# zyang1580/PDA

Hardware: AMD Instinct MI355X
Metric: users/sec full-catalogue top-K@50 (eval) (higher is better)
Workload: dtype f32; 1 GPU; C3: synthetic 1000000 users x 200000 items, d=128, PDA condition ((elu+1)*pop^0.22) head, masked top-K@50; ranks_seen=1

## Files before the change

pda_amd/csrc/pda_score_topk_v4.hip:

```cpp
#include "pda_v4_shared.h"
#include <cstdlib>
#include <type_traits>

using namespace pda_topk;

namespace {

constexpr int kCap4 = 57;
constexpr int kRing4 = 128;
constexpr int kWarmTiles = 4;
constexpr int kMainWaves = 8;
#ifndef PDA_W4_ABL
#define PDA_W4_ABL 0
#endif
#ifdef PDA_V4_PROF
__device__ unsigned long long pda_prof4[24];
#define PROF_T0(v) const long long v = __builtin_readcyclecounter()
#define PROF_T1(v, slot) prof[slot] += (unsigned long long)(__builtin_readcyclecounter() - v)
#define PROF_INC(slot, x) prof[slot] += (unsigned long long)(x)
#define PROF_FLUSH(first, last) do { if (lane == 0) for (int pq = (first); pq <= (last); ++pq) atomicAdd(&pda_prof4[pq], prof[pq]); } while (0)
#else
#define PROF_T0(v) do {} while (0)
#define PROF_T1(v, slot) do {} while (0)
#define PROF_INC(slot, x) do {} while (0)
// ... 634 lines not shown
            if (needa) ta = mna;
            if (needb) tb = mnb;
            for (int it = 0; it < 40; ++it) {
                const bool opena = needa && ca_t > cap_t && hia - ta > 1u;
                const bool openb = needb && cb_t > cap_t && hib - tb > 1u;
                if (!__any(opena || openb)) break;
                const uint32_t mida = opena ? ta + ((hia - ta) >> 1) : ta;
                const uint32_t midb = openb ? tb + ((hib - tb) >> 1) : tb;
                int cnta, cntb;
                count_ge2(mida, midb, cnta, cntb);
                if (opena) {
                    if (cnta >= K) {
                        ta = mida;
                        ca_t = cnta;
                    } else {
                        hia = mida;
                    }
                }
                if (openb) {
                    if (cntb >= K) {
                        tb = midb;
                        cb_t = cntb;
                    } else {
                        hib = midb;
                    }
                }
            }
        }
        emit_row(r, ta, ca_t);
        emit_row(r + 1, tb, cb_t);
    }
    pda_wave_sync();
    if (tid == 0) atomicAdd(reinterpret_cast<unsigned long long*>(g.stats + 2), (unsigned long long)(2 * nwarm));
    for (int rr = 0; rr < 32; ++rr) {
        uint64_t* buf = my_lists + rr * CAP;
        if (((PDA_W4_ABL & 4) == 0) && (g.warm_sorted || g.warm_final || (g.handover == nullptr && __builtin_amdgcn_readfirstlane(cntl[wave * 32 + rr]) > K)))
            compact_list<CAP>(buf, &cntl[wave * 32 + rr], &taul[wave * 32 + rr], K, lane);
        const int c = cntl[wave * 32 + rr];
        const int rb = utile * kUserTile + wave * 32 + rr;
        if (g.seed_out != nullptr) {
            uint32_t mn = lane < c ? (uint32_t)(buf[lane] >> 32) : 0xFFFFFFFFu;
#pragma unroll
            for (int o = 32; o >= 1; o >>= 1) mn = min(mn, (uint32_t)__shfl_xor((int)mn, o, 64));
            if (lane == 0 && rb < g.n_users_blk) g.seed_out[rb] = c >= K ? pda_unordf(mn) : -INFINITY;
        }
        if (g.kth_ws != nullptr) continue;
        if (g.handover != nullptr) {
            if (rb < g.n_users_blk && lane < CAP) g.handover[((size_t)split * g.n_users_blk + rb) * CAP + lane] = lane < c ? buf[lane] : 0ull;
            if (g.warm_final && rb < g.n_users_blk && lane < K) g.out_keys[((size_t)split * g.n_users_blk + rb) * K + lane] = lane < c ? buf[lane] : 0ull;
        } else if (rb < g.n_users_blk && lane < K) {
            const uint64_t k = lane < c ? buf[lane] : 0ull;
            g.out_keys[((size_t)split * g.n_users_blk + rb) * K + lane] = k;
        }
    }
    if (g.kth_ws != nullptr) {
        pda_wave_sync();
        const int rb0 = utile * kUserTile + wave * 32, nv = max(0, min(32, g.n_users_blk - rb0));
        if (lane < nv) {
            const uint64_t kl = my_lists[(size_t)lane * CAP + (K - 1)];
            g.kth_ws[(size_t)split * g.n_users_blk + rb0 + lane] = cntl[wave * 32 + lane] >= K ? pda_unordf((uint32_t)(kl >> 32)) : -INFINITY;
        }
        uint64_t* ob = g.out_keys + ((size_t)split * g.n_users_blk + rb0) * K;
        const int q64 = 64 / K, r64 = 64 % K;
        int rr = lane / K, p = lane % K;
        for (int i = lane; i < nv * K; i += 64) {
            ob[i] = p < cntl[wave * 32 + rr] ? my_lists[(size_t)rr * CAP + p] : 0ull;
            rr += q64;
            p += r64;
            if (p >= K) { p -= K; ++rr; }
        }
    }
    if (g.pred_ws != nullptr && lane < 32) {
        const int rb = utile * kUserTile + wave * 32 + lane;
        if (rb < g.n_users_blk) {
            g.pred_ws[2 * (size_t)rb] = predt[wave * 32 + lane];
            g.pred_ws[2 * (size_t)rb + 1] = nul[wave * 32 + lane];
        }
    }
}

constexpr int kWS5Waves = 8, kWS5Threads = 64 * kWS5Waves;
constexpr int kWarmPos = 64 * kWarmTiles;
constexpr size_t warm_score5_lds(int d) { return (size_t)kWarmPos * d * 4 + kWarmPos * 8 + (size_t)kWS5Waves * 32 * 2 * kWarmTiles * 4; }

template <int D, bool BF>
__global__ void __launch_bounds__(kWS5Threads) warm_score5_kernel(Args4 g) {
    extern __shared__ __attribute__((aligned(16))) unsigned char smem[];
    constexpr int RB = row_bytes(D);
    constexpr int NC = D / 8;
    constexpr int CPR4 = D / 4;
    float* Bt = reinterpret_cast<float*>(smem);
    float* popw = Bt + kWarmPos * D;
    int* idw = reinterpret_cast<int*>(popw + kWarmPos);
    unsigned* hmask = reinterpret_cast<unsigned*>(idw + kWarmPos);

    const int tid = threadIdx.x, lane = tid & 63, wave = tid >> 6;
    const int j = lane & 31, h = lane >> 5;
    const int nwarm = g.warm_tiles;
    const int npos = 64 * nwarm;
    for (int p = tid; p < npos; p += kWS5Threads) {
        const float* tl = reinterpret_cast<const float*>(g.rows + (size_t)p * RB + 2 * D + 32);
        popw[p] = tl[0];
        idw[p] = reinterpret_cast<const int*>(tl)[1];
    }
    __syncthreads();
    for (int id = tid; id < npos * CPR4; id += kWS5Threads) {
        const int jj = id / CPR4, ch = id % CPR4;
        *reinterpret_cast<f32x4*>(Bt + jj * D + 4 * (ch ^ swz<D>(jj & 31))) = pda_load4<BF>(g.I, (size_t)idw[jj] * D + 4 * ch);
    }
    if (blockIdx.x == 0) {
        for (int p = tid; p < kWarmPos; p += kWS5Threads) g.wscore[p] = p < npos ? (uint32_t)idw[p] : 0u;
        if (tid == 0) g.stats[8] = 5u;
    }
    __syncthreads();

    uint32_t* scores = g.wscore + kWarmPos;
    const int utiles_w = (g.n_users_blk + kUserTile - 1) / kUserTile;
    const int nunits = utiles_w * (kUserTile / 32);
    const int G = (int)gridDim.x, stride = G * kWS5Waves;
    unsigned* hm_l = hmask + wave * 32 * 2 * kWarmTiles;
    static_assert(2 * kWarmTiles == 8, "two 16-byte loads per row");

    auto row_uid = [&](int unit) -> int {
        const int rb = unit * 32 + j;
        return (unit < nunits && rb < g.n_users_blk) ? g.users[rb] : 0;
    };
    auto load_rows = [&](int unit_x, int uid, f32x4 (&a)[NC], u32x4& hm, bool& hm_on) __attribute__((always_inline)) {
        if (unit_x >= nunits) return;
        const int rb = unit_x * 32 + j;
#pragma unroll
        for (int c = 0; c < NC; ++c) a[c] = pda_load4<BF>(g.U, (size_t)uid * D + 4 * h + 8 * c);
        hm_on = false;
        if (g.hmask_tab != nullptr) {
            hm_on = rb < g.n_users_blk && (unsigned)uid < (unsigned)g.hmask_tab_rows;
            hm = *reinterpret_cast<const u32x4*>(g.hmask_tab + (size_t)(hm_on ? uid : 0) * (2 * kWarmTiles) + 4 * h);
        } else if (g.hmask_ws != nullptr) {
            hm_on = true;
            hm = *reinterpret_cast<const u32x4*>(g.hmask_ws + (size_t)rb * (2 * kWarmTiles) + 4 * h);
        }
    };
    unsigned long long n_tiles_done = 0ull;
    auto run_unit = [&](const int unit_in, f32x4 (&areg)[NC], const u32x4& hm_in, const bool hm_on) __attribute__((always_inline)) {
        const int unit = __builtin_amdgcn_readfirstlane(unit_in);
        const int row_blk = unit * 32 + j;
        if (unit * 32 + 32 > g.n_users_blk) {
            const f32x4 z = {0.f, 0.f, 0.f, 0.f};
#pragma unroll
            for (int c = 0; c < NC; ++c) areg[c] = row_blk < g.n_users_blk ? areg[c] : z;
        }
        const u32x4 hz = {0u, 0u, 0u, 0u};
        const u32x4 hmv = hm_on ? hm_in : hz;
        *reinterpret_cast<u32x4*>(hm_l + j * (2 * kWarmTiles) + 4 * h) = hmv;
        {
            constexpr int NK5 = D / 32;
            unsigned char* fb = g.ufrag_out + ((size_t)(row_blk >> 4) * (NK5 * 64) + (size_t)(row_blk & 15)) * 16 + 8 * h;
            float ssc[NC];
#pragma unroll
            for (int c = 0; c < NC; ++c) {
                const f32x4 v = areg[c];
                uint2 w;
                w.x = bf16_rne(v[0]) | (bf16_rne(v[1]) << 16);
                w.y = bf16_rne(v[2]) | (bf16_rne(v[3]) << 16);
                *reinterpret_cast<uint2*>(fb + ((c >> 2) * 64 + 16 * (c & 3)) * 16) = w;
                float ss = 0.f;
#pragma unroll
                for (int k = 0; k < 4; ++k) {
                    const float sq = v[k] * v[k];
                    ss += sq + __shfl_xor(sq, 32, 64);
                }
                ssc[c] = ss;
                __builtin_amdgcn_sched_barrier(0);
            }
#pragma unroll
            for (int o = NC / 2; o > 0; o >>= 1)
#pragma unroll
                for (int c = 0; c < o; ++c) ssc[c] += ssc[c + o];
            if (h == 0) g.unorm_out[row_blk] = sqrtf(ssc[0]) * 1.0009765625f * 1.0001f;
        }
        if ((unit & (kUserTile / 32 - 1)) == 0) n_tiles_done += (unsigned long long)(2 * nwarm);
        pda_wave_sync();
        const int j_lane = j, h_lane = h;
#pragma unroll 1
        for (int ht = 0; ht < 2 * nwarm; ++ht) {
            int j = j_lane, h = h_lane;
#if defined(__HIP_DEVICE_COMPILE__)
            asm volatile("" : "+v"(j), "+v"(h));
#endif
            const int bswz = swz<D>(j);
            const float* brow = Bt + (ht * 32 + j) * D;
            f32x16 acc0 = zero16v(), acc1 = zero16v();
            f32x4 b0 = *reinterpret_cast<const f32x4*>(brow + 4 * (h ^ bswz));
            f32x4 b1 = *reinterpret_cast<const f32x4*>(brow + 4 * ((2 + h) ^ bswz));
#pragma unroll
            for (int c = 0; c < NC; c += 2) {
                f32x4 n0 = b0, n1 = b1;
                if (c + 2 < NC) {
                    n0 = *reinterpret_cast<const f32x4*>(brow + 4 * ((2 * c + 4 + h) ^ bswz));
                    n1 = *reinterpret_cast<const f32x4*>(brow + 4 * ((2 * c + 6 + h) ^ bswz));
                }
#pragma unroll
                for (int q = 0; q < 4; ++q) {
                    acc0 = __builtin_amdgcn_mfma_f32_32x32x2f32(areg[c][q], b0[q], acc0, 0, 0, 0);
                    acc1 = __builtin_amdgcn_mfma_f32_32x32x2f32(areg[c + 1][q], b1[q], acc1, 0, 0, 0);
                }
                __builtin_amdgcn_sched_barrier(0);
                b0 = n0;
                b1 = n1;
            }
            const f32x16 accx = acc0 + acc1;
            const bool okw = (ht * 32 + j) < g.n_items_local;
            const float pv = popw[ht * 32 + j];
            const unsigned hb_mine = hm_l[j * (2 * kWarmTiles) + ht];
            const bool any_hb = __any(hb_mine != 0u);
            const uint32_t soff = (uint32_t)(unit * 32 + 4 * h) * (uint32_t)npos + (uint32_t)(ht * 32 + j);
#pragma unroll
            for (int r = 0; r < 16; ++r) {
                const int row = (r & 3) + 8 * (r >> 2) + 4 * h;
                float sc = accx[r];
                sc = (sc > 0.0f ? sc + 1.0f : __expf(sc)) * pv;
                bool p = okw && (sc >= -INFINITY);
                if (any_hb) {
                    const uint32_t hbr = (uint32_t)__shfl((int)hb_mine, row, 64);
                    if ((hbr >> j) & 1u) p = false;
                }
                scores[soff + (uint32_t)((r & 3) + 8 * (r >> 2)) * (uint32_t)npos] = p ? pda_ordf(sc + 0.0f) : 0u;
            }
        }
        pda_wave_sync();
    };
    int unit = (int)blockIdx.x + G * wave;
    f32x4 ra[NC], rb_[NC];
    u32x4 ha = {0u, 0u, 0u, 0u}, hb = {0u, 0u, 0u, 0u};
    bool oa = false, ob = false;
    load_rows(unit, row_uid(unit), ra, ha, oa);
    int uid_n = row_uid(unit + stride);
    while (unit < nunits) {
        load_rows(unit + stride, uid_n, rb_, hb, ob);
        uid_n = row_uid(unit + 2 * stride);
        run_unit(unit, ra, ha, oa);
        unit += stride;
        if (unit >= nunits) break;
        load_rows(unit + stride, uid_n, ra, ha, oa);
        uid_n = row_uid(unit + 2 * stride);
        run_unit(unit, rb_, hb, ob);
        unit += stride;
    }
    if (lane == 0 && n_tiles_done != 0ull) atomicAdd(reinterpret_cast<unsigned long long*>(g.stats + 2), n_tiles_done);
    if ((int)blockIdx.x == (nunits - 1) % G) {
        const size_t r0 = (size_t)utiles_w * kUserTile, r1 = ((size_t)g.n_users_blk + kUT5 - 1) / kUT5 * kUT5;
        const u32x4 z = {0u, 0u, 0u, 0u};
        for (size_t q = r0 * (2 * D) + (size_t)tid * 16; q < r1 * (2 * D); q += (size_t)kWS5Threads * 16) *reinterpret_cast<u32x4*>(g.ufrag_out + q) = z;
        for (size_t r = r0 + tid; r < r1; r += kWS5Threads) g.unorm_out[r] = 0.f;
    }
}

constexpr int kSelRows = 16;
__global__ void __launch_bounds__(256) __attribute__((amdgpu_waves_per_eu(8))) warm_select5_kernel(Args4 g) {
    constexpr int CAP = kCap4;
    __shared__ uint64_t lists[4][2][64];
    const int tid = threadIdx.x, lane = tid & 63, wave = tid >> 6;
    const int K = g.K, n = g.n_users_blk;
    const int npos = 64 * g.warm_tiles;
    const uint32_t* scores = g.wscore + kWarmPos;
    const int rb0 = ((int)blockIdx.x * 4 + wave) * kSelRows;
    if (rb0 >= n) return;
    const u32x4 idv = *reinterpret_cast<const u32x4*>(g.wscore + 4 * lane);
    uint32_t klo[4];
#pragma unroll
    for (int q = 0; q < 4; ++q) klo[q] = 0xFFFFFFFFu - (uint32_t)(g.item_offset + (int)idv[q]);
    const bool lane_on = 4 * lane < npos;
    float kth_mine = -INFINITY;

    auto count32 = [&](const u32x4& v, uint32_t t) __attribute__((always_inline)) -> int {
        return __popcll(__ballot(v[0] >= t)) + __popcll(__ballot(v[1] >= t)) + __popcll(__ballot(v[2] >= t)) + __popcll(__ballot(v[3] >= t));
    };
    auto key_of = [&](const u32x4& v, int q) __attribute__((always_inline)) -> uint64_t { return ((uint64_t)v[q] << 32) | (uint64_t)klo[q]; };
    auto count64 = [&](const u32x4& v, uint64_t t) __attribute__((always_inline)) -> int {
        int c = 0;
#pragma unroll
        for (int q = 0; q < 4; ++q) c += __popcll(__ballot(key_of(v, q) >= t));
        return c;
    };

#pragma unroll 1
    for (int it = 0; it < kSelRows; it += 2) {
        if (rb0 + it >= n) break;
        u32x4 v[2];
        uint32_t t[2], hi[2];
        int ct[2];
        bool need[2];
#pragma unroll
        for (int s = 0; s < 2; ++s) {
            const int rb = rb0 + it + s;
            const u32x4 z = {0u, 0u, 0u, 0u};
            v[s] = (lane_on && rb < n) ? *reinterpret_cast<const u32x4*>(scores + (size_t)rb * npos + 4 * lane) : z;
        }
#pragma unroll
        for (int s = 0; s < 2; ++s) {
            ct[s] = count32(v[s], 1u);
            t[s] = 1u;
            hi[s] = 0u;
            need[s] = ct[s] > CAP;
        }
        if (need[0] || need[1]) {
#pragma unroll
            for (int s = 0; s < 2; ++s) {
                uint32_t mx = max(max(v[s][0], v[s][1]), max(v[s][2], v[s][3])), mn = 0xFFFFFFFFu;
#pragma unroll
                for (int q = 0; q < 4; ++q) mn = min(mn, v[s][q] != 0u ? v[s][q] : 0xFFFFFFFFu);
#pragma unroll
                for (int o = 32; o >= 1; o >>= 1) {
                    mx = max(mx, (uint32_t)__shfl_xor((int)mx, o, 64));
                    mn = min(mn, (uint32_t)__shfl_xor((int)mn, o, 64));
                }
                hi[s] = (uint32_t)__builtin_amdgcn_readfirstlane((int)mx) + 1u;
                if (need[s]) t[s] = (uint32_t)__builtin_amdgcn_readfirstlane((int)mn);
            }
            for (int step = 0; step < 40; ++step) {
                const bool open0 = need[0] && ct[0] > CAP && hi[0] - t[0] > 1u;
                const bool open1 = need[1] && ct[1] > CAP && hi[1] - t[1] > 1u;
                if (!(open0 || open1)) break;
                const uint32_t mid0 = open0 ? t[0] + ((hi[0] - t[0]) >> 1) : t[0];
                const uint32_t mid1 = open1 ? t[1] + ((hi[1] - t[1]) >> 1) : t[1];
                const int c0 = count32(v[0], mid0), c1 = count32(v[1], mid1);
                if (open0) {
                    if (c0 >= K) { t[0] = mid0; ct[0] = c0; } else { hi[0] = mid0; }
                }
                if (open1) {
                    if (c1 >= K) { t[1] = mid1; ct[1] = c1; } else { hi[1] = mid1; }
                }
            }
        }
        uint64_t thr[2];
#pragma unroll
        for (int s = 0; s < 2; ++s) {
            thr[s] = (uint64_t)t[s] << 32;
// ... 964 lines not shown
        sh[t] += a;
        __syncthreads();
    }
    bins[t] = sh[t] - v;
}
__global__ void __launch_bounds__(1024) stop_scatter4_kernel(const int* __restrict__ bin_of, int* __restrict__ bins, int n, int32_t* __restrict__ perm) {
    __shared__ int sh[1024];
    const int t = threadIdx.x;
    sh[t] = 0;
    __syncthreads();
    int b[4], r[4];
    for (int i = 0; i < 4; ++i) {
        const int u = (int)blockIdx.x * 4096 + i * 1024 + t;
        b[i] = u < n ? bin_of[u] : -1;
        r[i] = b[i] >= 0 ? atomicAdd(&sh[b[i]], 1) : 0;
    }
    __syncthreads();
    const int c = sh[t];
    __syncthreads();
    sh[t] = c ? atomicAdd(&bins[t], c) : 0;
    __syncthreads();
    for (int i = 0; i < 4; ++i)
        if (b[i] >= 0) perm[sh[b[i]] + r[i]] = (int)blockIdx.x * 4096 + i * 1024 + t;
}

#include "pda_v5_sweep.h"

template <int D, int HEAD, bool BF, bool ES, int GM>
int launch_sweep4_kernel(const Args4& g, hipStream_t stream) {
    using G = Geo4<D, GM>;
    static char attr_done[kMaxDev4] = {};
    if (const int rc = dynamic_lds_once(reinterpret_cast<const void*>(&sweep4_kernel<D, HEAD, BF, ES, GM>), G::lds_total, attr_done)) return rc;
    const int utiles = (g.n_users_blk + G::UT - 1) / G::UT;
    hipLaunchKernelGGL((sweep4_kernel<D, HEAD, BF, ES, GM>), dim3((unsigned)(utiles * g.n_splits)), dim3(64 * G::WAVES), G::lds_total, stream, g);
    PDA_CHECK_LAUNCH();
    return PDA_OK;
}

template <int D, int HEAD, bool BF, int GM>
int launch_sweep4(const Args4& g, const Call4& c, hipStream_t stream) {
    if (!c.early_stop) return launch_sweep4_kernel<D, HEAD, BF, false, GM>(g, stream);
    if (!c.regroup) return launch_sweep4_kernel<D, HEAD, BF, true, GM>(g, stream);
    int* bins = g.regroup_ws;
    int* bin_of = bins + 1024;
    int32_t* perm = bin_of + g.n_users_blk;
    if (hipMemsetAsync(bins, 0, 1024 * sizeof(int), stream) != hipSuccess) return PDA_ERR_LAUNCH;
    hipLaunchKernelGGL((stop_predict4_kernel<D, BF>), dim3((unsigned)((g.n_users_blk + 31) / 32)), dim3(256), 0, stream, g, bin_of);
    const unsigned hb = (unsigned)((g.n_users_blk + 4095) / 4096);
    hipLaunchKernelGGL(stop_hist4_kernel, dim3(hb), dim3(1024), 0, stream, bin_of, g.n_users_blk, bins);
    hipLaunchKernelGGL(stop_scan4_kernel, dim3(1), dim3(1024), 0, stream, bins);
    hipLaunchKernelGGL(stop_scatter4_kernel, dim3(hb), dim3(1024), 0, stream, bin_of, bins, g.n_users_blk, perm);
    PDA_CHECK_LAUNCH();
    Args4 gp = g;
    gp.row_perm = perm;
    return launch_sweep4_kernel<D, HEAD, BF, true, GM>(gp, stream);
}

template <int D, int HEAD, bool BF>
int launch_warm4(const Args4& g, const Call4& c, hipStream_t stream) {
    Args4 gw = g;
    if (c.warm_whole) {
        gw.n_splits = 1;
        gw.warm_shared = 0;
    }
    const int utiles = (g.n_users_blk + kUserTile - 1) / kUserTile;
    if (c.mask_kernel) {
        hipLaunchKernelGGL(warm_mask4_kernel, dim3((unsigned)(utiles * gw.n_splits)), dim3(kThreads), 0, stream, gw, const_cast<uint32_t*>(g.hmask_ws));
        PDA_CHECK_LAUNCH();
    }
    if constexpr (HEAD == PDA_HEAD_POP && D <= 128) {
        if (c.warm == Call4::kWarmTwo) {
            constexpr size_t smem = warm_score5_lds(D);
            static char attr_done[kMaxDev4] = {};
            static int cu_of_dev[kMaxDev4] = {};
            int dev = 0;
            if (const int rc = dynamic_lds_once(reinterpret_cast<const void*>(&warm_score5_kernel<D, BF>), smem, attr_done, &dev)) return rc;
            if (cu_of_dev[dev] == 0) {
                int cus = 0;
                if (hipDeviceGetAttribute(&cus, hipDeviceAttributeMultiprocessorCount, dev) != hipSuccess || cus <= 0) return PDA_ERR_LAUNCH;
                cu_of_dev[dev] = cus;
            }
            const int n_cu = cu_of_dev[dev];
            const int nunits = utiles * (kUserTile / 32);
            hipLaunchKernelGGL((warm_score5_kernel<D, BF>), dim3((unsigned)(n_cu < nunits ? n_cu : nunits)), dim3(kWS5Threads), smem, stream, gw);
            PDA_CHECK_LAUNCH();
            hipLaunchKernelGGL(warm_select5_kernel, dim3((unsigned)((g.n_users_blk + 4 * kSelRows - 1) / (4 * kSelRows))), dim3(256), 0, stream, gw);
            PDA_CHECK_LAUNCH();
            return PDA_OK;
        }
    }
    if (c.warm != Call4::kWarm4) return PDA_ERR_ARG;
    constexpr size_t smem = 32 * D * 4 + (size_t)kUserTile * (kCap4 * 8 + 8) + kUserTile * 2 * kWarmTiles * 4 + 256 + kUserTile * 8;
    static char attr_done[kMaxDev4] = {};
    if (const int rc = dynamic_lds_once(reinterpret_cast<const void*>(&warm4_kernel<D, HEAD, BF>), smem, attr_done)) return rc;
    hipLaunchKernelGGL((warm4_kernel<D, HEAD, BF>), dim3((unsigned)(utiles * gw.n_splits)), dim3(kThreads), smem, stream, gw);
    PDA_CHECK_LAUNCH();
    return PDA_OK;
}

template <int D, int HEAD, bool BF>
int launch4(const Args4& g, const Call4& c, hipStream_t stream) {
    if (c.warm != Call4::kNoWarm) {
        if (const int rc = launch_warm4<D, HEAD, BF>(g, c, stream)) return rc;
    }
    if (c.sweep == Call4::kNoSweep || c.ends_in_warm) return PDA_OK;
    if constexpr (HEAD == PDA_HEAD_POP) {
        if (c.sweep == Call4::kSweep5) return launch_sweep5<D, BF, true, D == 256 ? 128 : 256>(g, c, stream);
    }
    if constexpr (D <= 128) {
        if (c.sweep == Call4::kSweep4Many) return launch_sweep4<D, HEAD, BF, 3>(g, c, stream);
    }
    if (c.sweep != Call4::kSweep4) return PDA_ERR_ARG;
    return launch_sweep4<D, HEAD, BF, 0>(g, c, stream);
}

int user_tile4(int d) { return d == 64 ? Geo4<64>::UT : d == 128 ? Geo4<128>::UT : Geo4<256>::UT; }
struct Ws4 {
    size_t tailrec, lists, bloom, hmask, regroup, handover, ufrag, unorm, seed, kth, wscore, total;
};
static Ws4 ws4_layout(int n_users_blk, int d, int n_splits) {
    auto al = [](size_t x) { return (x + 255) & ~(size_t)255; };
    Ws4 w{};
    w.tailrec = al(pda_score_topk_workspace_bytes(n_users_blk));
    w.lists = al(w.tailrec + ((size_t)n_users_blk + 511) / 512 * (size_t)n_splits * 8);
    size_t b = w.lists;
    const size_t ut = 1024;
    b += ((size_t)n_users_blk + ut - 1) / ut * (size_t)n_splits * ut * kCap4 * 8 + 256;
    w.bloom = al(b);
    w.hmask = al(w.bloom + (size_t)n_users_blk * 128);
    w.regroup = al(w.hmask + ((size_t)n_users_blk + kUserTile - 1) / kUserTile * (size_t)n_splits * kUserTile * 2 * kWarmTiles * 4);
    w.handover = al(w.regroup + (1024 + 4 * (size_t)n_users_blk) * 4);
    w.total = w.handover + (size_t)n_splits * (size_t)n_users_blk * kCap4 * 8;
    w.ufrag = al(w.total);
    w.unorm = w.ufrag;
    {
        const size_t n_pad = ((size_t)n_users_blk + kUT5 - 1) / kUT5 * kUT5;
        w.unorm = w.ufrag + al(n_pad * 2 * (size_t)d);
        w.total = w.unorm + al(n_pad * 4);
    }
    w.seed = w.total;
    w.total = w.seed + al((size_t)n_users_blk * 4);
    w.kth = w.total;
    w.total = w.kth + al((size_t)n_splits * (size_t)n_users_blk * 4);
    w.wscore = w.total;
    w.total = w.wscore + al((size_t)kWarmPos * 4 + ((size_t)n_users_blk + kUserTile - 1) / kUserTile * kUserTile * kWarmPos * 4);
    return w;
}
extern "C" size_t pda_score_topk4_workspace_bytes(int n_users_blk, int n_items_local, int d, int n_splits) {
    if (n_users_blk <= 0 || n_items_local <= 0 || (d != 64 && d != 128 && d != 256)) return 0;
    if (n_splits <= 0) n_splits = pda_score_topk4_auto_splits(n_users_blk, n_items_local, d);
    return ws4_layout(n_users_blk, d, n_splits).total;
}

int run_score4(const void* U, const void* I_shard, bool bf16, const void* prep, const float* pop_shard, const int32_t* users,
               int n_users_blk, int item_offset, int n_items_local, int d, const int64_t* hist_indptr, const int32_t* hist_indices,
               int hist_row_mode, int K, int head, int early_stop, int n_splits, uint64_t* out_keys, void* workspace, hipStream_t s,
               int phase = 3, const float* seed = nullptr, int warm_tiles = 0, const int* n_users_dev = nullptr,
               const uint32_t* mask_table = nullptr, int mask_table_rows = 0) {
    if (!U || !I_shard || !prep || !users || !out_keys || !workspace) return PDA_ERR_ARG;
    if (n_users_blk <= 0 || n_items_local <= 0 || item_offset < 0) return PDA_ERR_ARG;
    if (K < 1 || K > PDA_MAX_K) return PDA_ERR_ARG;
    if (early_stop < 0 || (early_stop & ~0x7FFF) != 0) return PDA_ERR_ARG;
    const bool warm_per_split = (early_stop & PDA_SWEEP_WARM_PER_SPLIT) != 0;
    const bool warm_one_kernel = (early_stop & PDA_SWEEP_WARM_ONE_KERNEL) != 0;
    const bool tail_share = (early_stop & PDA_SWEEP_TAIL_NO_SHARE) == 0;
    const bool tail_others_first = (early_stop & PDA_SWEEP_TAIL_OTHERS_FIRST) != 0, tail_min2 = (early_stop & PDA_SWEEP_TAIL_MIN2) != 0;
    int geometry = (early_stop & PDA_SWEEP_HUGE) ? 4 : (early_stop & PDA_SWEEP_MANY_CANDIDATES) ? 3 : 0;
// ... 175 lines not shown
    float a = -INFINITY, b = -INFINITY;
    for (int sp = 0; sp < S; ++sp) {
        const uint64_t* row = keys + ((size_t)sp * n_users + u) * K;
        const uint64_t ka = row[K - 1], kb = row[m - 1];
        if (ka != 0ull) a = fmaxf(a, pda_key_val(ka));
        if (kb != 0ull) b = fmaxf(b, pda_key_val(kb));
    }
    out[u] = a;
    out[(size_t)n_users + u] = b;
    out[2 * (size_t)n_users + u] = -b;
}
__device__ __forceinline__ float seed_thr(float lo, float hi, int j, int n_thr) {
    const bool open = lo > -INFINITY && hi < INFINITY && hi > lo;
    return open ? lo + (hi - lo) * ((float)(j + 1) / (float)(n_thr + 1)) : lo;
}
constexpr int kSeedThrMax = 15;
__global__ void __launch_bounds__(256) seed_counts_kernel(const uint64_t* __restrict__ keys, int S, int n_users, int K,
                                                          const float* __restrict__ bounds, int n_thr, int32_t* __restrict__ counts) {
    const int u = blockIdx.x * 256 + threadIdx.x;
    if (u >= n_users) return;
    const float lo = fmaxf(bounds[u], -bounds[2 * (size_t)n_users + u]), hi = bounds[(size_t)n_users + u];
    float thr[kSeedThrMax];
    int c[kSeedThrMax];
#pragma unroll
    for (int j = 0; j < kSeedThrMax; ++j) { thr[j] = seed_thr(lo, hi, j < n_thr ? j : 0, n_thr); c[j] = 0; }
    for (int sp = 0; sp < S; ++sp) {
        const uint64_t* row = keys + ((size_t)sp * n_users + u) * K;
        for (int q = 0; q < K; ++q) {
            const uint64_t k = row[q];
            if (k == 0ull) break;
            const float v = pda_key_val(k);
            if (v < thr[0]) break;
#pragma unroll
            for (int j = 0; j < kSeedThrMax; ++j) c[j] += (v >= thr[j]) ? 1 : 0;
        }
    }
#pragma unroll
    for (int j = 0; j < kSeedThrMax; ++j)
        if (j < n_thr) counts[(size_t)j * n_users + u] = c[j];
}
__global__ void __launch_bounds__(256) seed_pick_kernel(const float* __restrict__ bounds, const int32_t* __restrict__ counts, int n_thr,
                                                        int n_users, int K, float* __restrict__ seed) {
    const int u = blockIdx.x * 256 + threadIdx.x;
    if (u >= n_users) return;
    const float lo = fmaxf(bounds[u], -bounds[2 * (size_t)n_users + u]), hi = bounds[(size_t)n_users + u];
    float s = lo;
    for (int j = 0; j < n_thr; ++j)
        if (counts[(size_t)j * n_users + u] >= K) s = fmaxf(s, seed_thr(lo, hi, j, n_thr));
    seed[u] = s;
}

}

int pda_v4_run_score4_dev(const void* U, const void* I_shard, bool bf16, const void* prep, const float* pop_shard, const int32_t* users, int n_users_blk,
                          const int* n_users_dev, int item_offset, int n_items_local, int d, const int64_t* hist_indptr, const int32_t* hist_indices,
                          int hist_row_mode, int K, int head, int early_stop, int n_splits, const float* seed, uint64_t* out_keys, void* workspace, hipStream_t s) {
    return run_score4(U, I_shard, bf16, prep, pop_shard, users, n_users_blk, item_offset, n_items_local, d, hist_indptr, hist_indices, hist_row_mode, K, head,
                      early_stop, n_splits, out_keys, workspace, s, seed != nullptr ? 4 : 3, seed, 0, n_users_dev);
}

extern "C" int pda_topk_seed_bounds(const uint64_t* keys, int n_splits, int n_users_blk, int K, int m, float* bounds, void* stream) {
    if (!keys || !bounds || n_splits < 1 || n_users_blk < 1 || K < 1 || m < 1 || m > K) return PDA_ERR_ARG;
    hipLaunchKernelGGL(seed_bounds_kernel, dim3((unsigned)((n_users_blk + 255) / 256)), dim3(256), 0, reinterpret_cast<hipStream_t>(stream), keys,
                       n_splits, n_users_blk, K, m, bounds);
    PDA_CHECK_LAUNCH();
    return PDA_OK;
}
extern "C" int pda_topk_seed_counts(const uint64_t* keys, int n_splits, int n_users_blk, int K, const float* bounds, int n_thr, int32_t* counts,
                                    void* stream) {
    if (!keys || !bounds || !counts || n_splits < 1 || n_users_blk < 1 || K < 1 || n_thr < 1 || n_thr > kSeedThrMax) return PDA_ERR_ARG;
    hipLaunchKernelGGL(seed_counts_kernel, dim3((unsigned)((n_users_blk + 255) / 256)), dim3(256), 0, reinterpret_cast<hipStream_t>(stream), keys,
                       n_splits, n_users_blk, K, bounds, n_thr, counts);
    PDA_CHECK_LAUNCH();
    return PDA_OK;
}
extern "C" int pda_topk_seed_pick(const float* bounds, const int32_t* counts, int n_thr, int n_users_blk, int K, float* seed, void* stream) {
    if (!bounds || !seed || n_users_blk < 1 || K < 1 || n_thr < 0 || n_thr > kSeedThrMax || (n_thr > 0 && !counts)) return PDA_ERR_ARG;
    hipLaunchKernelGGL(seed_pick_kernel, dim3((unsigned)((n_users_blk + 255) / 256)), dim3(256), 0, reinterpret_cast<hipStream_t>(stream), bounds,
                       counts, n_thr, n_users_blk, K, seed);
    PDA_CHECK_LAUNCH();
    return PDA_OK;
}

#ifdef PDA_V5_EXITPROF
extern "C" int pda_debug_v5_exitprof(unsigned long long* out, int n_workgroups) {
    if (!out || n_workgroups < 1 || n_workgroups > kXpMaxWg) return PDA_ERR_ARG;
    if (hipMemcpyFromSymbol(out, HIP_SYMBOL(pda_v5_exitprof), (size_t)n_workgroups * 4 * kXpWords * sizeof(unsigned long long)) != hipSuccess) return PDA_ERR_LAUNCH;
    return PDA_OK;
}
extern "C" int pda_debug_v5_exitprof_words(void) { return kXpWords; }
extern "C" int pda_debug_v5_tail_pieces(int n) {
    if (n < 0) return PDA_ERR_ARG;
    if (hipMemcpyToSymbol(HIP_SYMBOL(pda_v5_tail_pieces), &n, sizeof(int)) != hipSuccess) return PDA_ERR_LAUNCH;
    return PDA_OK;
}
#endif
#ifdef PDA_V4_PROF
extern "C" int pda_debug_prof4(unsigned long long* out16, int reset) {
    if (hipMemcpyFromSymbol(out16, HIP_SYMBOL(pda_prof4), sizeof(unsigned long long) * 24) != hipSuccess) return PDA_ERR_LAUNCH;
    if (reset) { unsigned long long z[24] = {0}; if (hipMemcpyToSymbol(HIP_SYMBOL(pda_prof4), z, sizeof(z)) != hipSuccess) return PDA_ERR_LAUNCH; }
    return PDA_OK;
}
#endif

extern "C" int pda_score_topk4_auto_splits(int n_users_blk, int n_items_local, int d) {
    if (n_users_blk <= 0 || n_items_local <= 0) return 1;
    const int ut = user_tile4(d);
    const int utiles = (n_users_blk + ut - 1) / ut;
    const int n_tiles = (n_items_local + 63) / 64;
    int s = 1;
    while (utiles * s * 2 <= 256 && s < 64 && n_tiles / (s * 2) >= 3 * kWarmTiles) s *= 2;
    return s;
}

extern "C" size_t pda_item_prep4_bytes(int n_items_local, int d) { return n_items_local > 0 ? prep4_layout(n_items_local, d).total : 0; }

extern "C" int pda_item_prep4_f32(const float* I_shard, const float* pop_shard, const int32_t* order, int n_items_local, int d, void* prep,
                                  void* stream) {
    if (!I_shard || !prep || n_items_local <= 0) return PDA_ERR_ARG;
    return run_prep4(I_shard, false, pop_shard, order, n_items_local, d, prep, reinterpret_cast<hipStream_t>(stream));
}
extern "C" int pda_item_prep4_bf16(const uint16_t* I_shard, const float* pop_shard, const int32_t* order, int n_items_local, int d, void* prep,
                                   void* stream) {
    if (!I_shard || !prep || n_items_local <= 0) return PDA_ERR_ARG;
    return run_prep4(I_shard, true, pop_shard, order, n_items_local, d, prep, reinterpret_cast<hipStream_t>(stream));
}
extern "C" int pda_item_prep7_f32(const float* I_shard, const int32_t* order, int n_items_local, int d, void* prep, void* stream) {
    if (!I_shard || !prep || !order || n_items_local <= 0) return PDA_ERR_ARG;
    return run_prep4(I_shard, false, nullptr, order, n_items_local, d, prep, reinterpret_cast<hipStream_t>(stream), 1);
}
extern "C" int pda_item_prep7_bf16(const uint16_t* I_shard, const int32_t* order, int n_items_local, int d, void* prep, void* stream) {
    if (!I_shard || !prep || !order || n_items_local <= 0) return PDA_ERR_ARG;
    return run_prep4(I_shard, true, nullptr, order, n_items_local, d, prep, reinterpret_cast<hipStream_t>(stream), 1);
}
extern "C" int pda_item_prep4_check(const void* prep, int n_items_local, int d, void* stream) {
    if (!prep || n_items_local <= 0) return PDA_ERR_ARG;
    int bad = 0;
    hipStream_t s = reinterpret_cast<hipStream_t>(stream);
    if (hipMemcpyAsync(&bad, prep, 4, hipMemcpyDeviceToHost, s) != hipSuccess) return PDA_ERR_LAUNCH;
    if (hipStreamSynchronize(s) != hipSuccess) return PDA_ERR_LAUNCH;
    return bad ? PDA_ERR_ARG : PDA_OK;
}

extern "C" int pda_topk_kth_value(const uint64_t* keys, int n_splits, int n_users_blk, int K, int pos, float* out, void* stream) {
    if (!keys || !out || n_splits < 1 || n_users_blk < 1 || K < 1 || pos < 0 || pos >= K) return PDA_ERR_ARG;
    hipLaunchKernelGGL(kth_value_kernel, dim3((unsigned)((n_users_blk + 255) / 256)), dim3(256), 0, reinterpret_cast<hipStream_t>(stream), keys,
                       n_splits, n_users_blk, K, pos, out);
    PDA_CHECK_LAUNCH();
    return PDA_OK;
}

extern "C" int pda_topk_seed_refine(const uint64_t* keys, int n_splits, int n_users_blk, int K, float* lo, float* hi, float* mid,
                                    int32_t* counts, int mode, void* stream) {
    if (!keys || !lo || !hi || !mid || !counts || n_splits < 1 || n_users_blk < 1 || K < 1 || mode < 0 || mode > 2) return PDA_ERR_ARG;
    hipLaunchKernelGGL(seed_refine_kernel, dim3((unsigned)((n_users_blk + 255) / 256)), dim3(256), 0, reinterpret_cast<hipStream_t>(stream), keys,
                       n_splits, n_users_blk, K, lo, hi, mid, counts, mode);
    PDA_CHECK_LAUNCH();
    return PDA_OK;
}

extern "C" int pda_score_topk4_phase_f32(const float* U, const float* I_shard, const void* prep, const float* pop_shard, const int32_t* users,
                                         int n_users_blk, int item_offset, int n_items_local, int d, const int64_t* hist_indptr,
                                         const int32_t* hist_indices, int hist_row_mode, int K, int head, int early_stop, int n_splits,
                                         int phase, int warm_tiles, const float* seed, uint64_t* out_keys, void* workspace, void* stream) {
    if (phase != 1 && phase != 2 && phase != 4) return PDA_ERR_ARG;
    return run_score4(U, I_shard, false, prep, pop_shard, users, n_users_blk, item_offset, n_items_local, d, hist_indptr, hist_indices,
// ... 130 lines not shown
```

Before: 34.60 million users/s.

## Replace warm-score MFMA inner loop with hand-written assembly loop for D=128

For D=128 the warm-tile scoring loop in warm_score5_kernel is replaced by a hand-scheduled inline-assembly routine (WarmScoreLoop) that does the MFMA accumulation, popularity conditioning, masking and score stores. The aim is tighter instruction scheduling and less compiler overhead in the hottest loop. The cross-half shuffle in the norm reduction becomes a permlane32_swap, and lane indices are recomputed behind opaque asm to control register allocation. The change also adds optional timestamp instrumentation and an environment override for grid size. The new header is not shown, so correctness depends on external asm code.

```diff
diff --git a/pda_amd/csrc/pda_score_topk_v4.hip b/pda_amd/csrc/pda_score_topk_v4.hip
--- a/pda_amd/csrc/pda_score_topk_v4.hip
+++ b/pda_amd/csrc/pda_score_topk_v4.hip
@@ -740,6 +740,29 @@
 constexpr int kWS5Waves = 8, kWS5Threads = 64 * kWS5Waves;
 constexpr int kWarmPos = 64 * kWarmTiles;
 constexpr size_t warm_score5_lds(int d) { return (size_t)kWarmPos * d * 4 + kWarmPos * 8 + (size_t)kWS5Waves * 32 * 2 * kWarmTiles * 4; }
+#include "pda_warm_score_asm.h"
+template <int D>
+constexpr bool kWS5AsmLoop =
+#ifdef PDA_WS5_CPP_LOOP
+    false;
+#else
+    D == 128;
+#endif
+template <int N>
+struct WS5Set { static constexpr int value = N; };
+#ifdef PDA_WS5_STAMPS
+constexpr int kWspMaxWg = 512, kWspWords = 8;
+__device__ unsigned long long pda_ws5_stamps[kWspMaxWg * kWS5Waves * kWspWords];
+#define WSP(...) __VA_ARGS__
+__device__ __forceinline__ unsigned long long wsp_now() {
+    __builtin_amdgcn_sched_barrier(0);
+    const unsigned long long t = __builtin_readcyclecounter();
+    __builtin_amdgcn_sched_barrier(0);
+    return t;
+}
+#else
+#define WSP(...)
+#endif
 
 template <int D, bool BF>
 __global__ void __launch_bounds__(kWS5Threads) warm_score5_kernel(Args4 g) {
@@ -753,9 +776,9 @@
     unsigned* hmask = reinterpret_cast<unsigned*>(idw + kWarmPos);
 
     const int tid = threadIdx.x, lane = tid & 63, wave = tid >> 6;
-    const int j = lane & 31, h = lane >> 5;
     const int nwarm = g.warm_tiles;
     const int npos = 64 * nwarm;
+    WSP(unsigned long long wsp[kWspWords] = {}; const unsigned long long wsp_t0 = wsp_now(), wsp_r0 = __builtin_amdgcn_s_memrealtime();)
     for (int p = tid; p < npos; p += kWS5Threads) {
         const float* tl = reinterpret_cast<const float*>(g.rows + (size_t)p * RB + 2 * D + 32);
         popw[p] = tl[0];
@@ -771,6 +794,7 @@
         if (tid == 0) g.stats[8] = 5u;
     }
     __syncthreads();
+    WSP(wsp[0] = wsp_now() - wsp_t0;)
 
     uint32_t* scores = g.wscore + kWarmPos;
     const int utiles_w = (g.n_users_blk + kUserTile - 1) / kUserTile;
@@ -779,12 +803,21 @@
     unsigned* hm_l = hmask + wave * 32 * 2 * kWarmTiles;
     static_assert(2 * kWarmTiles == 8, "two 16-byte loads per row");
 
+    auto lane_now = [&]() __attribute__((always_inline)) -> int {
+        int l = lane;
+#if defined(__HIP_DEVICE_COMPILE__)
+        if constexpr (kWS5AsmLoop<D>) asm volatile("" : "+v"(l));
+#endif
+        return l;
+    };
     auto row_uid = [&](int unit) -> int {
+        const int j = lane_now() & 31;
         const int rb = unit * 32 + j;
         return (unit < nunits && rb < g.n_users_blk) ? g.users[rb] : 0;
     };
     auto load_rows = [&](int unit_x, int uid, f32x4 (&a)[NC], u32x4& hm, bool& hm_on) __attribute__((always_inline)) {
         if (unit_x >= nunits) return;
+        const int ln = lane_now(), j = ln & 31, h = ln >> 5;
         const int rb = unit_x * 32 + j;
 #pragma unroll
         for (int c = 0; c < NC; ++c) a[c] = pda_load4<BF>(g.U, (size_t)uid * D + 4 * h + 8 * c);
@@ -798,9 +831,11 @@
         }
     };
     unsigned long long n_tiles_done = 0ull;
-    auto run_unit = [&](const int unit_in, f32x4 (&areg)[NC], const u32x4& hm_in, const bool hm_on) __attribute__((always_inline)) {
+    auto run_unit = [&](auto set_c, const int unit_in, f32x4 (&areg)[NC], const u32x4& hm_in, const bool hm_on) __attribute__((always_inline)) {
         const int unit = __builtin_amdgcn_readfirstlane(unit_in);
+        const int ln = lane_now(), j = ln & 31, h = ln >> 5;
         const int row_blk = unit * 32 + j;
+        WSP(const unsigned long long wsp_u0 = wsp_now();)
         if (unit * 32 + 32 > g.n_users_blk) {
             const f32x4 z = {0.f, 0.f, 0.f, 0.f};
 #pragma unroll
@@ -823,8 +858,12 @@
                 float ss = 0.f;
 #pragma unroll
                 for (int k = 0; k < 4; ++k) {
-                    const float sq = v[k] * v[k];
-                    ss += sq + __shfl_xor(sq, 32, 64);
+                    float sq = v[k] * v[k];
+#if defined(__HIP_DEVICE_COMPILE__)
+                    if constexpr (kWS5AsmLoop<D>) asm volatile("" : "+v"(sq));
+#endif
+                    const auto sw = __builtin_amdgcn_permlane32_swap(__float_as_uint(sq), __float_as_uint(sq), false, false);
+                    ss += sq + __uint_as_float(h ? sw[0] : sw[1]);
                 }
                 ssc[c] = ss;
                 __builtin_amdgcn_sched_barrier(0);
@@ -837,9 +876,23 @@
         }
         if ((unit & (kUserTile / 32 - 1)) == 0) n_tiles_done += (unsigned long long)(2 * nwarm);
         pda_wave_sync();
+        WSP(wsp[1] += wsp_now() - wsp_u0; wsp[5] += 1ull;)
+        if constexpr (kWS5AsmLoop<D>) {
+            const unsigned bt_lds = (unsigned)(size_t)(__attribute__((address_space(3))) unsigned char*)reinterpret_cast<unsigned char*>(Bt);
+            const unsigned pop_lds = (unsigned)(size_t)(__attribute__((address_space(3))) unsigned char*)reinterpret_cast<unsigned char*>(popw);
+            const unsigned hm_lds = (unsigned)(size_t)(__attribute__((address_space(3))) unsigned char*)reinterpret_cast<unsigned char*>(hm_l);
+            WSP(const unsigned long long wsp_a0 = wsp_now();)
+            WarmScoreLoop<D, decltype(set_c)::value>::run(areg, (unsigned)(j * (D * 4) + 16 * ((h ^ j) & 15)), bt_lds, hm_lds + (unsigned)(4 * h * 2 * kWarmTiles * 4),
+                                                          pop_lds + 4u * (unsigned)j, 1u << j, j, 4u * ((unsigned)(4 * h) * (unsigned)npos + (unsigned)j),
+                                                          scores + (size_t)unit * 32 * (size_t)npos, 4u * (unsigned)npos, nwarm, g.n_items_local);
+            WSP(wsp[2] += wsp_now() - wsp_a0; wsp[6] += (unsigned long long)(2 * nwarm);)
+            pda_wave_sync();
+            return;
+        }
         const int j_lane = j, h_lane = h;
 #pragma unroll 1
         for (int ht = 0; ht < 2 * nwarm; ++ht) {
+            WSP(const unsigned long long wsp_h0 = wsp_now();)
             int j = j_lane, h = h_lane;
 #if defined(__HIP_DEVICE_COMPILE__)
             asm volatile("" : "+v"(j), "+v"(h));
@@ -865,6 +918,7 @@
                 b0 = n0;
                 b1 = n1;
             }
+            WSP(const unsigned long long wsp_h1 = wsp_now(); wsp[2] += wsp_h1 - wsp_h0;)
             const f32x16 accx = acc0 + acc1;
             const bool okw = (ht * 32 + j) < g.n_items_local;
             const float pv = popw[ht * 32 + j];
@@ -883,6 +937,7 @@
                 }
                 scores[soff + (uint32_t)((r & 3) + 8 * (r >> 2)) * (uint32_t)npos] = p ? pda_ordf(sc + 0.0f) : 0u;
             }
+            WSP(wsp[3] += wsp_now() - wsp_h1; wsp[6] += 1ull;)
         }
         pda_wave_sync();
     };
@@ -895,12 +950,12 @@
     while (unit < nunits) {
         load_rows(unit + stride, uid_n, rb_, hb, ob);
         uid_n = row_uid(unit + 2 * stride);
-        run_unit(unit, ra, ha, oa);
+        run_unit(WS5Set<0>{}, unit, ra, ha, oa);
         unit += stride;
         if (unit >= nunits) break;
         load_rows(unit + stride, uid_n, ra, ha, oa);
         uid_n = row_uid(unit + 2 * stride);
-        run_unit(unit, rb_, hb, ob);
+        run_unit(WS5Set<1>{}, unit, rb_, hb, ob);
         unit += stride;
     }
     if (lane == 0 && n_tiles_done != 0ull) atomicAdd(reinterpret_cast<unsigned long long*>(g.stats + 2), n_tiles_done);
@@ -910,6 +965,8 @@
         for (size_t q = r0 * (2 * D) + (size_t)tid * 16; q < r1 * (2 * D); q += (size_t)kWS5Threads * 16) *reinterpret_cast<u32x4*>(g.ufrag_out + q) = z;
         for (size_t r = r0 + tid; r < r1; r += kWS5Threads) g.unorm_out[r] = 0.f;
     }
+    WSP(wsp[4] = wsp_now() - wsp_t0; wsp[7] = __builtin_amdgcn_s_memrealtime() - wsp_r0;
+        if (lane == 0 && blockIdx.x < (unsigned)kWspMaxWg) for (int q = 0; q < kWspWords; ++q) pda_ws5_stamps[((size_t)blockIdx.x * kWS5Waves + wave) * kWspWords + q] = wsp[q];)
 }
 
 constexpr int kSelRows = 16;
@@ -2040,7 +2097,12 @@
             }
             const int n_cu = cu_of_dev[dev];
             const int nunits = utiles * (kUserTile / 32);
-            hipLaunchKernelGGL((warm_score5_kernel<D, BF>), dim3((unsigned)(n_cu < nunits ? n_cu : nunits)), dim3(kWS5Threads), smem, stream, gw);
+            int grid = n_cu < nunits ? n_cu : nunits;
+            if (const char* cap = getenv("PDA_WARM_SCORE_GRID")) {
+                const int c = atoi(cap);
+                if (c >= 1 && c < grid) grid = c;
+            }
+            hipLaunchKernelGGL((warm_score5_kernel<D, BF>), dim3((unsigned)grid), dim3(kWS5Threads), smem, stream, gw);
             PDA_CHECK_LAUNCH();
             hipLaunchKernelGGL(warm_select5_kernel, dim3((unsigned)((g.n_users_blk + 4 * kSelRows - 1) / (4 * kSelRows))), dim3(256), 0, stream, gw);
             PDA_CHECK_LAUNCH();
@@ -2382,6 +2444,13 @@
     return PDA_OK;
 }
 
+#ifdef PDA_WS5_STAMPS
+extern "C" int pda_debug_ws5_stamps(unsigned long long* out, int n_workgroups) {
+    if (!out || n_workgroups < 1 || n_workgroups > kWspMaxWg) return PDA_ERR_ARG;
+    if (hipMemcpyFromSymbol(out, HIP_SYMBOL(pda_ws5_stamps), (size_t)n_workgroups * kWS5Waves * kWspWords * sizeof(unsigned long long)) != hipSuccess) return PDA_ERR_LAUNCH;
+    return PDA_OK;
+}
+#endif
 #ifdef PDA_V5_EXITPROF
 extern "C" int pda_debug_v5_exitprof(unsigned long long* out, int n_workgroups) {
     if (!out || n_workgroups < 1 || n_workgroups > kXpMaxWg) return PDA_ERR_ARG;
```

Result: no change. 34.69 million users/s, median of 6 (+0.2%).
